# kasvii/PMCE

Measured on AMD Instinct MI355X. Metric: 16-frame clips/s, higher is better.
Workload: dtype f32; 1 GPU; full two-stream PMCE forward (temporal pose encoder + CoEvoDecoder + 6890-vertex upsample + J_regressor), batch=256/GPU, T=16, J=17, C=512, random-init weights; global_batch=256, seq_len=16, joints=17, embed_dim=512, parallelism=clip-sharded dp1, weights replicated, gemm_mode=split_f16, streams=4, batches_enqueued_ahead=2, lanes=staggered

## Files before the change

### pmce_amd/csrc/coevo.hip

```cpp
#include "common.hpp"

#define NV 431
#define ND 64
#define NTILE 14
#define LDW64 68
#define LDW256 260

__global__ __launch_bounds__(256) void vertex_init_gather_kernel(const float* __restrict__ joints,
                                                                 const int* __restrict__ vj, float* __restrict__ vt, int B,
                                                                 int J) {
  const int idx = blockIdx.x * blockDim.x + threadIdx.x;
  if (idx >= B * NV * 3) return;
  const int l = idx % 3, v = (idx / 3) % NV, b = idx / (3 * NV);
  vt[idx] = joints[((long long)b * J + vj[v]) * 3 + l];
}

#define JLD 65

#define JWL 68
#define JS_THREADS 512
struct JTile {
  f32x4 r[2];
};
__device__ __forceinline__ void jtile_fetch(JTile& t, const float* __restrict__ W, int ld, int n0, int k0, int tid) {
#pragma unroll
  for (int q = 0; q < 2; ++q) {
    const int row = (tid >> 4) + 32 * q, c4 = tid & 15;
    t.r[q] = *reinterpret_cast<const f32x4*>(W + (long long)(n0 + row) * ld + k0 + 4 * c4);
  }
}
__device__ __forceinline__ void jtile_store(float* s_w, const JTile& t, int tid) {
#pragma unroll
  for (int q = 0; q < 2; ++q) {
    const int row = (tid >> 4) + 32 * q, c4 = tid & 15;
    *reinterpret_cast<f32x4*>(s_w + row * JWL + 4 * c4) = t.r[q];
  }
}
template <int KIN, int NOUT>
__device__ __forceinline__ void lin_tiled(const float* in, int ild, const float* __restrict__ W, const float* __restrict__ b, float* out,
                                          int old, int J, int tid, bool gelu, float* s_w, JTile& pre, const float* __restrict__ Wnext,
                                          int ldnext) {
  constexpr int NT = NOUT / 64, KT = KIN / 64;
  const int lane = tid & 63, tg = tid >> 6;
#pragma unroll 1
  for (int nt = 0; nt < NT; ++nt) {
    float acc[4] = {0.f, 0.f, 0.f, 0.f};
    const int n = nt * 64 + lane;
    const float bn = b[n];
#pragma unroll 1
    for (int kt = 0; kt < KT; ++kt) {
      __syncthreads();
      jtile_store(s_w, pre, tid);
      __syncthreads();
      if (kt + 1 < KT) jtile_fetch(pre, W, KIN, nt * 64, (kt + 1) * 64, tid);
      else if (nt + 1 < NT) jtile_fetch(pre, W, KIN, (nt + 1) * 64, 0, tid);
      else if (Wnext) jtile_fetch(pre, Wnext, ldnext, 0, 0, tid);
      const float* wrow = s_w + lane * JWL;
#pragma unroll 4
      for (int k4 = 0; k4 < 16; ++k4) {
        const f32x4 wv = *reinterpret_cast<const f32x4*>(wrow + 4 * k4);
#pragma unroll
        for (int t = 0; t < 4; ++t) {
          const int i = tg + 8 * t;
          if (i < J) {
            const float* x = in + i * ild + kt * 64 + 4 * k4;
            acc[t] = fmaf(wv.x, x[0], acc[t]);
            acc[t] = fmaf(wv.y, x[1], acc[t]);
            acc[t] = fmaf(wv.z, x[2], acc[t]);
            acc[t] = fmaf(wv.w, x[3], acc[t]);
          }
        }
      }
    }
#pragma unroll
    for (int t = 0; t < 4; ++t) {
      const int i = tg + 8 * t;
      if (i < J) {
        const float v = acc[t] + bn;
        out[i * old + n] = gelu ? gelu_erf(v) : v;
      }
    }
  }
}
__device__ __forceinline__ void adaln_small8(const float* in, float* out, const float* __restrict__ gb, int J, int tid) {
  const int lane = tid & 63, wave = tid >> 6;
  const float gam = gb[lane], bet = gb[64 + lane];
  for (int i = wave; i < J; i += 8) {
    const float x = in[i * JLD + lane];
    const float mean = wave_sum(x) * (1.0f / 64.0f);
    const float d = x - mean;
    const float var = wave_sum(d * d) * (1.0f / 63.0f);
    float sd = sqrtf(var);
    if (var == INFINITY) {
      int e = 0;
      frexpf(wave_max(fabsf(d)), &e);
      const float ds = ldexpf(d, -e);
      sd = ldexpf(sqrtf(wave_sum(ds * ds) * (1.0f / 63.0f)), e);
    }
    out[i * JLD + lane] = gam * d / (sd + 1e-6f) + bet;
  }
}

#define CAM_VLD 52
#define CA_IMG_HDR 68
#define CA_IMG_FLOATS(J) (CA_IMG_HDR + 2 * (J) * LDW64 + 64 * CAM_VLD)
#define CA_IMG_STRIDE 6528
struct CaFoldArgs {
  const float *xk, *xv;
  const float *jt, *Wj, *bj, *jpos, *Wj2v, *bj2v, *j2vK;
  float* jf_out;
  const float* GB;
  int gb_stride, iq, ik, iv;
  const float *Wq, *bq, *Wk, *bk, *Wv, *bv, *Wp;
  float *Kf, *s0, *Vf;
  float* img;
  int J;
};
__global__ __launch_bounds__(JS_THREADS) void ca_fold_kernel(CaFoldArgs a) {
  __shared__ float s_a[32 * JLD];
  __shared__ float s_b[32 * JLD];
  __shared__ float s_k[32 * JLD];
  __shared__ float s_v[32 * JLD];
  __shared__ __attribute__((aligned(16))) float s_w[64 * JWL];
  __shared__ __attribute__((aligned(16))) float s_wp[64 * JWL];
  __shared__ __attribute__((aligned(16))) float s_img[CA_IMG_STRIDE];
  __shared__ float s_red[16];
  const int b = blockIdx.x, tid = threadIdx.x, lane = tid & 63, wave = tid >> 6;
  const int J = a.J;
  const float* gb = a.GB + (long long)b * a.gb_stride;
  JTile pre, prep;
  jtile_fetch(pre, a.xk ? a.Wk : a.Wj2v, 64, 0, 0, tid);
  jtile_fetch(prep, a.Wp, 64, 0, 0, tid);
  const float gq = gb[a.iq * 128 + lane], bqv = gb[a.iq * 128 + 64 + lane];
  if (a.img)
    for (int i = tid; i < CA_IMG_STRIDE; i += JS_THREADS) s_img[i] = 0.f;
  if (a.xk) {
    for (int idx = tid; idx < J * 64; idx += JS_THREADS) {
      const int i = idx >> 6, c = idx & 63;
      s_a[i * JLD + c] = a.xk[((long long)b * J + i) * 64 + c];
      s_b[i * JLD + c] = a.xv[((long long)b * J + i) * 64 + c];
    }
    jtile_store(s_wp, prep, tid);
    __syncthreads();
  } else {
    const int c = tid & 63, i0 = tid >> 6;
    const float w0 = a.Wj[c * 3], w1 = a.Wj[c * 3 + 1], w2 = a.Wj[c * 3 + 2], bjc = a.bj[c];
    float px[4], py[4], pz[4], pe[4], ke[4];
#pragma unroll
    for (int u = 0; u < 4; ++u) {
      const int i = i0 + 8 * u;
      if (i < J) {
        const float* p = a.jt + ((long long)b * J + i) * 3;
        px[u] = p[0]; py[u] = p[1]; pz[u] = p[2];
        pe[u] = a.jpos[i * 64 + c];
        ke[u] = a.j2vK[i * 64 + c];
      }
    }
#pragma unroll
    for (int u = 0; u < 4; ++u) {
      const int i = i0 + 8 * u;
      if (i < J) {
        const float v = ((w0 * px[u] + w1 * py[u] + w2 * pz[u]) + bjc) + pe[u];
        s_b[i * JLD + c] = v;
        if (a.jf_out) a.jf_out[((long long)b * J + i) * 64 + c] = v;
      }
    }
    jtile_store(s_wp, prep, tid);
    lin_tiled<64, 64>(s_b, JLD, a.Wj2v, a.bj2v, s_k, JLD, J, tid, false, s_w, pre, a.Wk, 64);
    __syncthreads();
#pragma unroll
    for (int u = 0; u < 4; ++u) {
      const int i = i0 + 8 * u;
      if (i < J) s_a[i * JLD + c] = s_k[i * JLD + c] + ke[u];
    }
    __syncthreads();
  }
  adaln_small8(s_a, s_k, gb + a.ik * 128, J, tid);
  adaln_small8(s_b, s_v, gb + a.iv * 128, J, tid);
  lin_tiled<64, 64>(s_k, JLD, a.Wk, a.bk, s_a, JLD, J, tid, false, s_w, pre, a.Wv, 64);
  lin_tiled<64, 64>(s_v, JLD, a.Wv, a.bv, s_b, JLD, J, tid, false, s_w, pre, a.Wq, 64);
  __syncthreads();
  jtile_store(s_w, pre, tid);
  __syncthreads();
  const float scale = 0.17677669529663688110f * 1.44269504088896340736f;
  float* Kfb = a.Kf ? a.Kf + (long long)b * 64 * 64 : nullptr;
  float* Vfb = a.Vf ? a.Vf + (long long)b * 64 * 64 : nullptr;
  float* s0b = a.s0 ? a.s0 + (long long)b * 64 : nullptr;
  float kfr[8], vfr[8];
  float mk = 0.f, mv = 0.f;
#pragma unroll
  for (int q8 = 0; q8 < 8; ++q8) {
    const int row = wave + 8 * q8;
    const int h = row >> 5, i = row & 31;
    float kf = 0.f, vf = 0.f, sc = 0.f;
    if (i < J) {
      float M = 0.f;
#pragma unroll
      for (int q = 0; q < 8; ++q) {
        const f32x4 wp4 = *reinterpret_cast<const f32x4*>(s_wp + lane * JWL + 32 * h + 4 * q);
        const float* kd = s_a + i * JLD + 32 * h + 4 * q;
        const float* vd = s_b + i * JLD + 32 * h + 4 * q;
        const float* wq = s_w + (32 * h + 4 * q) * JWL + lane;
        M += wq[0] * kd[0];
        vf += vd[0] * wp4.x;
        M += wq[JWL] * kd[1];
        vf += vd[1] * wp4.y;
        M += wq[2 * JWL] * kd[2];
        vf += vd[2] * wp4.z;
        M += wq[3 * JWL] * kd[3];
        vf += vd[3] * wp4.w;
      }
      kf = scale * gq * M;
      float t = bqv * M;
      if (lane < 32) t += a.bq[32 * h + lane] * s_a[i * JLD + 32 * h + lane];
      sc = scale * wave_sum(t);
    }
    if (Kfb) Kfb[row * 64 + lane] = kf;
    if (Vfb) Vfb[lane * 64 + row] = vf;
    if (s0b && lane == 0) s0b[row] = sc;
    if (a.img && lane == 0) s_img[row] = sc;
    kfr[q8] = kf;
    vfr[q8] = vf;
    mk = fmaxf(mk, fabsf(kf));
    mv = fmaxf(mv, fabsf(vf));
  }
  if (!a.img) return;
  mk = wave_max(mk);
  mv = wave_max(mv);
  if (lane == 0) {
    s_red[wave] = mk;
    s_red[8 + wave] = mv;
  }
  __syncthreads();
  float MK = 0.f, MV = 0.f;
#pragma unroll
  for (int w = 0; w < 8; ++w) {
    MK = fmaxf(MK, s_red[w]);
    MV = fmaxf(MV, s_red[8 + w]);
  }
  int ek = 0, ev = 0;
  const bool sk = MK > 0.f && MK < INFINITY, sv = MV > 0.f && MV < INFINITY;
  if (sk) frexpf(MK, &ek);
  if (sv) frexpf(MV, &ev);
  const float upK = sk ? ldexpf(1.f, 15 - ek) : 1.f, upV = sv ? ldexpf(1.f, 15 - ev) : 1.f;
  if (tid == 0) {
    s_img[64] = (sk ? ldexpf(1.f, ek - 15) : 1.f) * 0.0009765625f;
    s_img[65] = (sv ? ldexpf(1.f, ev - 15) : 1.f) * 0.0009765625f;
  }
  _Float16* im = reinterpret_cast<_Float16*>(s_img);
#pragma unroll
  for (int q8 = 0; q8 < 8; ++q8) {
    const int row = wave + 8 * q8;
    const int h = row >> 5, i = row & 31;
    if (i < J) {
      const float v = pinned(kfr[q8] * upK);
      const _Float16 hi = (_Float16)v, lo = (_Float16)(v - (float)hi);
      const int c = lane, ks = c >> 4, hbb = (c >> 2) & 1, e = (c & 3) + 4 * ((c >> 3) & 1);
      const int idx = (CA_IMG_HDR + (h * J + i) * LDW64) * 2 + ((ks * 2 + hbb) * 2) * 8 + e;
      im[idx] = hi;
      im[idx + 8] = lo;
    }
    if (i < 24) {
      const float v = pinned(vfr[q8] * upV);
      const _Float16 hi = (_Float16)v, lo = (_Float16)(v - (float)hi);
      const int base = (CA_IMG_HDR + 2 * J * LDW64 + lane * CAM_VLD) * 2 + h * 48;
      if (i < 16) {
        const int idx = base + ((i >> 2) & 1) * 16 + (i & 3) + 4 * (i >> 3);
        im[idx] = hi;
        im[idx + 8] = lo;
      } else {
        const int jj = i - 16;
        const int idx = base + 32 + (jj >> 2) * 8 + (jj & 3);
        im[idx] = hi;
        im[idx + 4] = lo;
      }
    }
  }
  __syncthreads();
  float* dst = a.img + (long long)b * CA_IMG_STRIDE;
  for (int i4 = tid; i4 < CA_IMG_FLOATS(J) / 4; i4 += JS_THREADS) reinterpret_cast<f32x4*>(dst)[i4] = reinterpret_cast<const f32x4*>(s_img)[i4];
}

__global__ __launch_bounds__(448, 4) void vertex_ca_kernel(const float* __restrict__ xq, const float* __restrict__ vt,
                                                        const float* __restrict__ Wv3, const float* __restrict__ Eq,
                                                        const float* __restrict__ Kf, const float* __restrict__ s0,
                                                        const float* __restrict__ Vf, const float* __restrict__ bp,
                                                        float* __restrict__ out, int J) {
  __shared__ __attribute__((aligned(16))) float sK[64 * LDW64];
  __shared__ __attribute__((aligned(16))) float sV[64 * LDW64];
  __shared__ float sS0[64];
  const int b = blockIdx.y, tid = threadIdx.x;
  const int lane = tid & 63, wave = tid >> 6;
  const int n0 = lane & 31, hb = lane >> 5;
  const int tile = blockIdx.x * 7 + wave;
// ... 1191 lines not shown
        }
#pragma unroll
        for (int r = 0; r < 16; ++r) y[16 * nt + r] = fmaf(fmaf(c[r], 0.00048828125f, m[r]), down, add[16 * nt + r]);
      }
    } else {
      f32x16 t[2];
#pragma unroll
      for (int nt = 0; nt < 2; ++nt)
#pragma unroll
        for (int r = 0; r < 16; ++r) t[nt][r] = add[16 * nt + r];
      tl_gemm<8, 2, LDW64>(sw, x, t, n0, hb);
#pragma unroll
      for (int nt = 0; nt < 2; ++nt)
#pragma unroll
        for (int r = 0; r < 16; ++r) y[16 * nt + r] = t[nt][r];
    }
  };
  for (int wt = blockIdx.x * 4 + wave; wt < ntiles; wt += gridDim.x * 4) {
    const int b = wt / NTILE, tile = wt % NTILE;
    const int v = tile * 32 + n0;
    const bool valid = v < NV;
    const int vc = valid ? v : NV - 1;
    const long long tok = (long long)b * NV + vc;
    float xk[32], xv[32];
    if (xk_in) {
      load_slots(xk_in + tok * 64, xk, hb);
      load_slots(xv_in + tok * 64, xv, hb);
    } else {
      const float* p = vt + tok * 3;
      const float p0 = p[0], p1 = p[1], p2 = p[2];
      load_slots(Ev + (long long)vc * 64, xv, hb);
#pragma unroll
      for (int s = 0; s < 32; ++s) {
        const int c = slot_channel(s, hb);
        xv[s] = (Wv3[c * 3] * p0 + Wv3[c * 3 + 1] * p1 + Wv3[c * 3 + 2] * p2) + xv[s];
      }
      float e[32];
      load_slots(Ek + (long long)vc * 64, e, hb);
      linear64(sW2, 0, xv, e, xk);
    }
    const float* gb = GB + (long long)b * gb_stride;
    float a[32], bias[32], y[32];
    adaln_slots(xk, a, gb + ik * 128, hb);
#pragma unroll
    for (int s = 0; s < 32; ++s) bias[s] = bk[slot_channel(s, hb)];
    linear64(sWk, 1, a, bias, y);
    if (valid) store_slots(kv + tok * 128, y, hb);
    adaln_slots(xv, a, gb + iv * 128, hb);
#pragma unroll
    for (int s = 0; s < 32; ++s) bias[s] = bv[slot_channel(s, hb)];
    linear64(sWv, 2, a, bias, y);
    if (valid) store_slots(kv + tok * 128 + 64, y, hb);
  }
}
__global__ __launch_bounds__(256) void tkv_pack_kernel(const float* __restrict__ W2, const float* __restrict__ Wk, const float* __restrict__ Wv,
                                                       float* __restrict__ img) {
  __shared__ float red[16];
  const float* W[3] = {W2, Wk, Wv};
  for (int i = 0; i < 3; ++i) {
    float up, down;
    weight_scale(W[i], 64 * 64, red, threadIdx.x, 256, up, down);
    stage_weight_split<64>(img + i * 64 * LDW64, W[i], 64, up, threadIdx.x, 256);
    if (threadIdx.x == 0) {
      img[3 * 64 * LDW64 + 2 * i] = up;
      img[3 * 64 * LDW64 + 2 * i + 1] = down;
    }
  }
}

struct JointStreamW {
  const float *wq, *bq, *proj_w, *proj_b;
  const float *fc1_w, *fc1_b, *fc2_w, *fc2_b;
  const float *qkv_w, *qkv_b, *sproj_w, *sproj_b;
  const float *sfc1_w, *sfc1_b, *sfc2_w, *sfc2_b;
  const float *coor_w, *coor_b;
  int i_normq, i_norm2, i_snorm1, i_snorm2;
};

__global__ __launch_bounds__(JS_THREADS) void joint_stream_kernel(const float* __restrict__ xq_in, const float* __restrict__ jQ,
                                                                  const float* __restrict__ kv, const float* __restrict__ GB,
                                                                  int gb_stride, JointStreamW w, const float* __restrict__ jt,
                                                                  float* __restrict__ y_out, float* __restrict__ pose_out, int J,
                                                                  int stage) {
  __shared__ float s_y[32 * JLD];
  __shared__ float s_a[32 * JLD];
  __shared__ float s_q[32 * JLD];
  __shared__ __attribute__((aligned(16))) float s_h[32 * 257];
  __shared__ __attribute__((aligned(16))) float s_kv[64 * 128];
  __shared__ __attribute__((aligned(16))) float s_w[64 * JWL];
  __shared__ float s_gb[4 * 128];
  __shared__ float s_cw[3 * 64 + 3];
  const int b = blockIdx.x, tid = threadIdx.x;
  {
    const float* gbg = GB + (long long)b * gb_stride;
    const int inst = tid >> 7, c = tid & 127;
    const int ii = inst == 0 ? w.i_normq : inst == 1 ? w.i_norm2 : inst == 2 ? w.i_snorm1 : w.i_snorm2;
    s_gb[inst * 128 + c] = gbg[ii * 128 + c];
    if (tid < 192) s_cw[tid] = w.coor_w[tid];
    if (tid < 3) s_cw[192 + tid] = w.coor_b[tid];
  }
  JTile pre;
  if (stage != 4) jtile_fetch(pre, w.wq, 64, 0, 0, tid);
  else jtile_fetch(pre, w.qkv_w, 64, 0, 0, tid);
  for (int idx = tid; idx < J * 64; idx += JS_THREADS) {
    const int i = idx >> 6, c = idx & 63;
    float v = xq_in[((long long)b * J + i) * 64 + c];
    if (jQ) v += jQ[i * 64 + c];
    s_y[i * JLD + c] = v;
  }
  __syncthreads();
  if (stage != 4) {
    adaln_small8(s_y, s_a, s_gb + 0 * 128, J, tid);
    lin_tiled<64, 64>(s_a, JLD, w.wq, w.bq, s_q, JLD, J, tid, false, s_w, pre, w.proj_w, 64);
    __syncthreads();
    {
      const int P = J * 8, NSL = JS_THREADS / P;
      const int pr = tid % P, sl = tid / P;
      const int i = pr >> 3, h = pr & 7;
      const bool act = sl < NSL;
      float qv[8], o[8];
      const float scale = 0.35355339059327376220f * 1.44269504088896340736f;
#pragma unroll
      for (int d = 0; d < 8; ++d) {
        qv[d] = act ? s_q[i * JLD + 8 * h + d] * scale : 0.f;
        o[d] = 0.f;
      }
      float m = -INFINITY, l = 0.f;
      const float* kvb = kv + (long long)b * NV * 128;
      f32x4 kvr[4];
      auto kv_fetch = [&](int j0) {
        const int nj = min(64, NV - j0);
#pragma unroll
        for (int q = 0; q < 4; ++q) {
          const int idx = tid + q * JS_THREADS, r = idx >> 5, c4 = idx & 31;
          if (r < nj) kvr[q] = *reinterpret_cast<const f32x4*>(kvb + (long long)(j0 + r) * 128 + 4 * c4);
        }
      };
      kv_fetch(0);
      for (int j0 = 0; j0 < NV; j0 += 64) {
        const int nj = min(64, NV - j0);
        __syncthreads();
#pragma unroll
        for (int q = 0; q < 4; ++q) {
          const int idx = tid + q * JS_THREADS, r = idx >> 5, c4 = idx & 31;
          if (r < nj) *reinterpret_cast<f32x4*>(&s_kv[r * 128 + 4 * c4]) = kvr[q];
        }
        __syncthreads();
        if (j0 + 64 < NV) kv_fetch(j0 + 64);
        if (act) {
          for (int r0 = sl; r0 < nj; r0 += 4 * NSL) {
            float sc[4];
#pragma unroll
            for (int u = 0; u < 4; ++u) {
              const int r = r0 + u * NSL;
              if (r < nj) {
                const f32x4 k0 = *reinterpret_cast<const f32x4*>(&s_kv[r * 128 + 8 * h]);
                const f32x4 k1 = *reinterpret_cast<const f32x4*>(&s_kv[r * 128 + 8 * h + 4]);
                sc[u] = qv[0] * k0.x + qv[1] * k0.y + qv[2] * k0.z + qv[3] * k0.w + qv[4] * k1.x + qv[5] * k1.y + qv[6] * k1.z +
                        qv[7] * k1.w;
              } else {
                sc[u] = -INFINITY;
              }
            }
            const float mn = fmaxf(fmaxf(m, fmaxf(sc[0], sc[1])), fmaxf(sc[2], sc[3]));
            const float corr = __builtin_amdgcn_exp2f(m - mn);
            l *= corr;
#pragma unroll
            for (int d = 0; d < 8; ++d) o[d] *= corr;
#pragma unroll
            for (int u = 0; u < 4; ++u) {
              const int r = r0 + u * NSL;
              if (r < nj) {
                const float pj = __builtin_amdgcn_exp2f(sc[u] - mn);
                l += pj;
                const f32x4 v0 = *reinterpret_cast<const f32x4*>(&s_kv[r * 128 + 64 + 8 * h]);
                const f32x4 v1 = *reinterpret_cast<const f32x4*>(&s_kv[r * 128 + 64 + 8 * h + 4]);
                o[0] += pj * v0.x;
                o[1] += pj * v0.y;
                o[2] += pj * v0.z;
                o[3] += pj * v0.w;
                o[4] += pj * v1.x;
                o[5] += pj * v1.y;
                o[6] += pj * v1.z;
                o[7] += pj * v1.w;
              }
            }
            m = mn;
          }
        }
      }
      if (act) {
        float* st = s_h + (sl * P + pr) * 10;
        st[0] = m;
        st[1] = l;
#pragma unroll
        for (int d = 0; d < 8; ++d) st[2 + d] = o[d];
      }
      __syncthreads();
      if (act && sl == 0) {
        float M = m;
        for (int s2 = 1; s2 < NSL; ++s2) M = fmaxf(M, s_h[(s2 * P + pr) * 10]);
        float L = 0.f, O[8] = {0.f, 0.f, 0.f, 0.f, 0.f, 0.f, 0.f, 0.f};
        for (int s2 = 0; s2 < NSL; ++s2) {
          const float* st = s_h + (s2 * P + pr) * 10;
          const float c = __builtin_amdgcn_exp2f(st[0] - M);
          L += st[1] * c;
#pragma unroll
          for (int d = 0; d < 8; ++d) O[d] += st[2 + d] * c;
        }
        const float inv = 1.0f / L;
#pragma unroll
        for (int d = 0; d < 8; ++d) s_a[i * JLD + 8 * h + d] = O[d] * inv;
      }
    }
    lin_tiled<64, 64>(s_a, JLD, w.proj_w, w.proj_b, s_q, JLD, J, tid, false, s_w, pre, stage == 1 ? nullptr : w.fc1_w, 64);
    __syncthreads();
    for (int idx = tid; idx < J * 64; idx += JS_THREADS) {
      const int i = idx >> 6, c = idx & 63;
      s_y[i * JLD + c] += s_q[i * JLD + c];
    }
    __syncthreads();
    if (stage == 1) {
      for (int idx = tid; idx < J * 64; idx += JS_THREADS) y_out[(long long)b * J * 64 + idx] = s_y[(idx >> 6) * JLD + (idx & 63)];
      return;
    }
    adaln_small8(s_y, s_a, s_gb + 1 * 128, J, tid);
    lin_tiled<64, 256>(s_a, JLD, w.fc1_w, w.fc1_b, s_h, 257, J, tid, true, s_w, pre, w.fc2_w, 256);
    lin_tiled<256, 64>(s_h, 257, w.fc2_w, w.fc2_b, s_q, JLD, J, tid, false, s_w, pre, stage == 2 ? nullptr : w.qkv_w, 64);
    __syncthreads();
    for (int idx = tid; idx < J * 64; idx += JS_THREADS) {
      const int i = idx >> 6, c = idx & 63;
      s_y[i * JLD + c] += s_q[i * JLD + c];
    }
    __syncthreads();
    if (stage == 2) {
      for (int idx = tid; idx < J * 64; idx += JS_THREADS) y_out[(long long)b * J * 64 + idx] = s_y[(idx >> 6) * JLD + (idx & 63)];
      return;
    }
  }
  adaln_small8(s_y, s_a, s_gb + 2 * 128, J, tid);
  lin_tiled<64, 192>(s_a, JLD, w.qkv_w, w.qkv_b, s_h, 193, J, tid, false, s_w, pre, w.sproj_w, 64);
  __syncthreads();
  {
    const int i = tid >> 3, h = tid & 7;
    if (i < J) {
      const float scale = 0.35355339059327376220f * 1.44269504088896340736f;
      float qv[8], o[8];
#pragma unroll
      for (int d = 0; d < 8; ++d) {
        qv[d] = s_h[i * 193 + 8 * h + d] * scale;
        o[d] = 0.f;
      }
      float m = -INFINITY, l = 0.f;
      for (int j = 0; j < J; ++j) {
        float sc = 0.f;
#pragma unroll
        for (int d = 0; d < 8; ++d) sc += qv[d] * s_h[j * 193 + 64 + 8 * h + d];
        const float mn = fmaxf(m, sc);
        const float corr = __builtin_amdgcn_exp2f(m - mn), pj = __builtin_amdgcn_exp2f(sc - mn);
        l = l * corr + pj;
#pragma unroll
        for (int d = 0; d < 8; ++d) o[d] = o[d] * corr + pj * s_h[j * 193 + 128 + 8 * h + d];
        m = mn;
      }
      const float inv = 1.0f / l;
#pragma unroll
      for (int d = 0; d < 8; ++d) s_a[i * JLD + 8 * h + d] = o[d] * inv;
    }
  }
  lin_tiled<64, 64>(s_a, JLD, w.sproj_w, w.sproj_b, s_q, JLD, J, tid, false, s_w, pre, w.sfc1_w, 64);
  __syncthreads();
  for (int idx = tid; idx < J * 64; idx += JS_THREADS) {
    const int i = idx >> 6, c = idx & 63;
    s_y[i * JLD + c] += s_q[i * JLD + c];
  }
  __syncthreads();
  adaln_small8(s_y, s_a, s_gb + 3 * 128, J, tid);
  lin_tiled<64, 256>(s_a, JLD, w.sfc1_w, w.sfc1_b, s_h, 257, J, tid, true, s_w, pre, w.sfc2_w, 256);
  lin_tiled<256, 64>(s_h, 257, w.sfc2_w, w.sfc2_b, s_q, JLD, J, tid, false, s_w, pre, nullptr, 0);
  __syncthreads();
  for (int idx = tid; idx < J * 64; idx += JS_THREADS) {
    const int i = idx >> 6, c = idx & 63;
    s_y[i * JLD + c] += s_q[i * JLD + c];
  }
  __syncthreads();
  if (y_out)
    for (int idx = tid; idx < J * 64; idx += JS_THREADS) y_out[(long long)b * J * 64 + idx] = s_y[(idx >> 6) * JLD + (idx & 63)];
  if (pose_out) {
    for (int idx = tid; idx < J * 3; idx += JS_THREADS) {
      const int i = idx / 3, k = idx % 3;
      float s = 0.f;
      for (int c = 0; c < 64; ++c) s += s_cw[k * 64 + c] * s_y[i * JLD + c];
      pose_out[((long long)b * J + i) * 3 + k] = (s + s_cw[192 + k]) + jt[((long long)b * J + i) * 3 + k];
    }
  }
}

template <bool PACKED>
__global__ __launch_bounds__(256) void build_final_operand_kernel(const float* __restrict__ g, const float* __restrict__ vt,
                                                                  float* __restrict__ A, int B, int KP) {
  const long long idx = (long long)blockIdx.x * blockDim.x + threadIdx.x;
  if (idx >= (long long)B * KP) return;
  const int b = (int)(idx / KP), k = (int)(idx % KP);
  float v = 0.f;
  if (k < 2048)
    v = fmaxf(g[(long long)b * 2048 + k], 0.f);
  else if (k < 2048 + NV * 3)
    v = vt[(long long)b * NV * 3 + (k - 2048)];
  if constexpr (PACKED) {
    _Float16* row = reinterpret_cast<_Float16*>(A + (long long)b * KP);
    const _Float16 h = (_Float16)v;
    row[(k >> 4) * 32 + (k & 15)] = h;
    row[(k >> 4) * 32 + 16 + (k & 15)] = lo_plane_plain(v, h);
  } else {
    A[idx] = v;
  }
}

__global__ __launch_bounds__(256) void j_regress_kernel(const float* __restrict__ mesh, const int* __restrict__ indptr,
                                                        const int* __restrict__ indices, const float* __restrict__ data,
                                                        float* __restrict__ out, int B, int R, int NVF, float scale) {
  const int idx = blockIdx.x * blockDim.x + threadIdx.x;
  if (idx >= B * R * 3) return;
  const int l = idx % 3, j = (idx / 3) % R, b = idx / (3 * R);
  const float* m = mesh + (long long)b * NVF * 3;
  float s = 0.f;
  for (int e = indptr[j]; e < indptr[j + 1]; ++e) s += data[e] * (m[(long long)indices[e] * 3 + l] * scale);
  out[idx] = s;
}

#define MLP_WAVES 8
#define CAM_WAVES 7
static int mlp_grid(int B) {
  const int tiles = B * NTILE;
  int g = (tiles + MLP_WAVES - 1) / MLP_WAVES;
  return g < 256 ? g : 256;
}
static int tl_grid(int B, int per_cu) {
  const int tiles = B * NTILE;
  int g = (tiles + 3) / 4;
  const int cap = 256 * per_cu;
  return g < cap ? g : cap;
}

extern "C" int pmce_vertex_init_gather_f32(const float* joints, const int* vj, float* vt, int B, int J, hipStream_t stream) {
  PMCE_REQUIRE(joints && vj && vt && B > 0 && J > 0, "vertex_init_gather: bad args");
  const int n = B * NV * 3;
  hipLaunchKernelGGL(vertex_init_gather_kernel, dim3((n + 255) / 256), dim3(256), 0, stream, joints, vj, vt, B, J);
  return pmce_check_launch("vertex_init_gather");
}

static int launch_ca_fold(const CaFoldArgs& a, int B, hipStream_t stream, const char* what) {
  PMCE_REQUIRE(a.J >= 1 && a.J <= 32 && B > 0, "%s: J must be in 1..32", what);
  PMCE_REQUIRE(!a.img || (a.J <= 23 && (reinterpret_cast<uintptr_t>(a.img) & 15) == 0), "%s: the f16 image needs J <= 23 and a 16-byte aligned buffer", what);
  hipLaunchKernelGGL(ca_fold_kernel, dim3(B), dim3(JS_THREADS), 0, stream, a);
  return pmce_check_launch(what);
}
extern "C" int pmce_ca_image_floats(void) { return CA_IMG_STRIDE; }
extern "C" int pmce_ca_image_floats_written(int J) { return CA_IMG_FLOATS(J); }
extern "C" int pmce_ca_fold_f32(const float* xk, const float* xv, const float* GB, int gb_stride, int iq, int ik, int iv,
                                const float* Wq, const float* bq, const float* Wk, const float* bk, const float* Wv,
                                const float* bv, const float* Wp, float* Kf, float* s0, float* Vf, float* img, int B, int J,
                                hipStream_t stream) {
  PMCE_REQUIRE(xk && xv && GB && Wq && bq && Wk && bk && Wv && bv && Wp, "ca_fold: null pointer");
  CaFoldArgs a{};
  a.xk = xk; a.xv = xv; a.GB = GB; a.gb_stride = gb_stride; a.iq = iq; a.ik = ik; a.iv = iv;
  a.Wq = Wq; a.bq = bq; a.Wk = Wk; a.bk = bk; a.Wv = Wv; a.bv = bv; a.Wp = Wp;
// ... 186 lines not shown
```

Before: 30570 clips/s.

## Move joint-stream linears to FP32 MFMA with async LDS weight DMA

Swaps the scalar-FMA tiled linear layers in the cross-attention fold and joint-stream kernels for 32x32x2 FP32 MFMA tiles. Full weight matrices are prefetched into LDS through buffer-load-to-LDS DMA ahead of use, replacing the register-staged tile double buffering. The FFN keeps its hidden activations in registers and feeds them straight into the second GEMM. K-split partial sums are reduced in shared memory with the bias and residual fused in. The LDS is reorganised into one aliased arena and token rows are padded to 32 with zeros, which raises LDS footprint and could lower occupancy.

After: 30740 clips/s (median of 6 runs). No clear change (+0.6%).

```diff
diff --git a/pmce_amd/csrc/coevo.hip b/pmce_amd/csrc/coevo.hip
--- a/pmce_amd/csrc/coevo.hip
+++ b/pmce_amd/csrc/coevo.hip
@@ -15,70 +15,88 @@
   vt[idx] = joints[((long long)b * J + vj[v]) * 3 + l];
 }
 
-#define JLD 65
+#define JLD 68
 
 #define JWL 68
+#define JWL4 260
 #define JS_THREADS 512
-struct JTile {
-  f32x4 r[2];
-};
-__device__ __forceinline__ void jtile_fetch(JTile& t, const float* __restrict__ W, int ld, int n0, int k0, int tid) {
-#pragma unroll
-  for (int q = 0; q < 2; ++q) {
-    const int row = (tid >> 4) + 32 * q, c4 = tid & 15;
-    t.r[q] = *reinterpret_cast<const f32x4*>(W + (long long)(n0 + row) * ld + k0 + 4 * c4);
-  }
-}
-__device__ __forceinline__ void jtile_store(float* s_w, const JTile& t, int tid) {
-#pragma unroll
-  for (int q = 0; q < 2; ++q) {
-    const int row = (tid >> 4) + 32 * q, c4 = tid & 15;
-    *reinterpret_cast<f32x4*>(s_w + row * JWL + 4 * c4) = t.r[q];
-  }
-}
-template <int KIN, int NOUT>
-__device__ __forceinline__ void lin_tiled(const float* in, int ild, const float* __restrict__ W, const float* __restrict__ b, float* out,
-                                          int old, int J, int tid, bool gelu, float* s_w, JTile& pre, const float* __restrict__ Wnext,
-                                          int ldnext) {
-  constexpr int NT = NOUT / 64, KT = KIN / 64;
-  const int lane = tid & 63, tg = tid >> 6;
-#pragma unroll 1
-  for (int nt = 0; nt < NT; ++nt) {
-    float acc[4] = {0.f, 0.f, 0.f, 0.f};
-    const int n = nt * 64 + lane;
+#define JW_SLOT (64 * JWL)
+template <int KIN>
+__device__ __forceinline__ void jl_dma_rows(float* lds_dst, const float* __restrict__ W, int rows, int tid) {
+  constexpr int CPR = KIN / 4 + 1;
+  const __amdgpu_buffer_rsrc_t rsrc = __builtin_amdgcn_make_buffer_rsrc(const_cast<float*>(W), 0, 0xffffffff, 0x00020000);
+  const unsigned base = __builtin_amdgcn_readfirstlane((unsigned)(uintptr_t)(const __attribute__((address_space(3))) float*)lds_dst);
+  const int w0 = __builtin_amdgcn_readfirstlane(tid >> 6), lane = tid & 63;
+  const int pieces = rows * CPR / 64;
+  for (int c = w0; c < pieces; c += JS_THREADS / 64) {
+    const int g = c * 64 + lane, row = g / CPR, col = min(g % CPR, CPR - 2);
+    lds_dma16(rsrc, (unsigned)((row * KIN + 4 * col) * 4), 0, base + (unsigned)c * 1024u);
+  }
+}
+template <int NQ>
+__device__ __forceinline__ void jl_mma(f32x16& acc, const float* Wrow, const float* xrow) {
+#pragma unroll
+  for (int q = 0; q < NQ; ++q) {
+    const f32x4 wv = *reinterpret_cast<const f32x4*>(Wrow + 8 * q);
+    const f32x4 xv = *reinterpret_cast<const f32x4*>(xrow + 8 * q);
+    acc = __builtin_amdgcn_mfma_f32_32x32x2f32(wv.x, xv.x, acc, 0, 0, 0);
+    acc = __builtin_amdgcn_mfma_f32_32x32x2f32(wv.y, xv.y, acc, 0, 0, 0);
+    acc = __builtin_amdgcn_mfma_f32_32x32x2f32(wv.z, xv.z, acc, 0, 0, 0);
+    acc = __builtin_amdgcn_mfma_f32_32x32x2f32(wv.w, xv.w, acc, 0, 0, 0);
+  }
+}
+__device__ __forceinline__ f32x16 jl_zero() {
+  f32x16 z;
+#pragma unroll
+  for (int r = 0; r < 16; ++r) z[r] = 0.f;
+  return z;
+}
+__device__ __forceinline__ void jl_store_part(float* part, int nb, const f32x16& acc, int lane) {
+  const int tok = lane & 31, hb = lane >> 5;
+#pragma unroll
+  for (int r = 0; r < 16; ++r) part[(32 * nb + (r & 3) + 8 * (r >> 2) + 4 * hb) * 32 + tok] = acc[r];
+}
+__device__ __forceinline__ void jl_lin64_parts(const float* in, const float* Wl, float* parts, int tid) {
+  const int lane = tid & 63, wave = tid >> 6, n = lane & 31, hb = lane >> 5;
+  const int nb = wave & 1, kq = wave >> 1;
+  f32x16 acc = jl_zero();
+  jl_mma<2>(acc, Wl + (32 * nb + n) * JWL + 16 * kq + 4 * hb, in + n * JLD + 16 * kq + 4 * hb);
+  jl_store_part(parts + kq * 2048, nb, acc, lane);
+}
+template <int NP>
+__device__ __forceinline__ void jl_meet(const float* parts, const float* __restrict__ b, float* out, bool residual, int J, int tid) {
+#pragma unroll
+  for (int u = 0; u < 4; ++u) {
+    const int o = tid + JS_THREADS * u, n = o >> 5, tok = o & 31;
     const float bn = b[n];
-#pragma unroll 1
-    for (int kt = 0; kt < KT; ++kt) {
-      __syncthreads();
-      jtile_store(s_w, pre, tid);
-      __syncthreads();
-      if (kt + 1 < KT) jtile_fetch(pre, W, KIN, nt * 64, (kt + 1) * 64, tid);
-      else if (nt + 1 < NT) jtile_fetch(pre, W, KIN, (nt + 1) * 64, 0, tid);
-      else if (Wnext) jtile_fetch(pre, Wnext, ldnext, 0, 0, tid);
-      const float* wrow = s_w + lane * JWL;
-#pragma unroll 4
-      for (int k4 = 0; k4 < 16; ++k4) {
-        const f32x4 wv = *reinterpret_cast<const f32x4*>(wrow + 4 * k4);
-#pragma unroll
-        for (int t = 0; t < 4; ++t) {
-          const int i = tg + 8 * t;
-          if (i < J) {
-            const float* x = in + i * ild + kt * 64 + 4 * k4;
-            acc[t] = fmaf(wv.x, x[0], acc[t]);
-            acc[t] = fmaf(wv.y, x[1], acc[t]);
-            acc[t] = fmaf(wv.z, x[2], acc[t]);
-            acc[t] = fmaf(wv.w, x[3], acc[t]);
-          }
-        }
-      }
-    }
-#pragma unroll
-    for (int t = 0; t < 4; ++t) {
-      const int i = tg + 8 * t;
-      if (i < J) {
-        const float v = acc[t] + bn;
-        out[i * old + n] = gelu ? gelu_erf(v) : v;
-      }
+    float s = parts[o];
+#pragma unroll
+    for (int p = 1; p < NP; ++p) s += parts[p * 2048 + o];
+    const float v = s + bn;
+    if (tok < J) out[tok * JLD + n] = residual ? out[tok * JLD + n] + v : v;
+  }
+}
+__device__ __forceinline__ void jl_ffn_parts(const float* in, const float* W1l, const float* W2l, const float* __restrict__ b1, f32x16* acc2,
+                                             int tid) {
+  const int lane = tid & 63, wave = tid >> 6, n = lane & 31, hb = lane >> 5;
+  float bv[16];
+#pragma unroll
+  for (int r = 0; r < 16; ++r) bv[r] = b1[32 * wave + (r & 3) + 8 * (r >> 2) + 4 * hb];
+  f32x16 h = jl_zero();
+  jl_mma<8>(h, W1l + (32 * wave + n) * JWL + 4 * hb, in + n * JLD + 4 * hb);
+#pragma unroll
+  for (int r = 0; r < 16; ++r) h[r] = gelu_erf(h[r] + bv[r]);
+#pragma unroll
+  for (int nb = 0; nb < 2; ++nb) {
+    acc2[nb] = jl_zero();
+    const float* Wrow = W2l + (32 * nb + n) * JWL4 + 32 * wave + 4 * hb;
+#pragma unroll
+    for (int q = 0; q < 4; ++q) {
+      const f32x4 wv = *reinterpret_cast<const f32x4*>(Wrow + 8 * q);
+      acc2[nb] = __builtin_amdgcn_mfma_f32_32x32x2f32(wv.x, h[4 * q + 0], acc2[nb], 0, 0, 0);
+      acc2[nb] = __builtin_amdgcn_mfma_f32_32x32x2f32(wv.y, h[4 * q + 1], acc2[nb], 0, 0, 0);
+      acc2[nb] = __builtin_amdgcn_mfma_f32_32x32x2f32(wv.z, h[4 * q + 2], acc2[nb], 0, 0, 0);
+      acc2[nb] = __builtin_amdgcn_mfma_f32_32x32x2f32(wv.w, h[4 * q + 3], acc2[nb], 0, 0, 0);
     }
   }
 }
@@ -117,30 +135,36 @@
   int J;
 };
 __global__ __launch_bounds__(JS_THREADS) void ca_fold_kernel(CaFoldArgs a) {
-  __shared__ float s_a[32 * JLD];
-  __shared__ float s_b[32 * JLD];
-  __shared__ float s_k[32 * JLD];
-  __shared__ float s_v[32 * JLD];
-  __shared__ __attribute__((aligned(16))) float s_w[64 * JWL];
-  __shared__ __attribute__((aligned(16))) float s_wp[64 * JWL];
-  __shared__ __attribute__((aligned(16))) float s_img[CA_IMG_STRIDE];
-  __shared__ float s_red[16];
+  __shared__ __attribute__((aligned(16))) float smem[4 * 32 * JLD + 5 * JW_SLOT + 2 * JW_SLOT + 16];
+  float* s_a = smem;
+  float* s_b = s_a + 32 * JLD;
+  float* s_k = s_b + 32 * JLD;
+  float* s_v = s_k + 32 * JLD;
+  float* s_wt = s_v + 32 * JLD;
+  float* s_wq = s_wt + 3 * JW_SLOT;
+  float* s_wp = s_wt + 4 * JW_SLOT;
+  float* s_parts = s_wt + 5 * JW_SLOT;
+  float* s_M = s_parts;
+  float* s_VF = s_parts + JW_SLOT;
+  float* s_red = s_parts + 2 * JW_SLOT;
+  float* s_img = s_wt;
   const int b = blockIdx.x, tid = threadIdx.x, lane = tid & 63, wave = tid >> 6;
   const int J = a.J;
   const float* gb = a.GB + (long long)b * a.gb_stride;
-  JTile pre, prep;
-  jtile_fetch(pre, a.xk ? a.Wk : a.Wj2v, 64, 0, 0, tid);
-  jtile_fetch(prep, a.Wp, 64, 0, 0, tid);
+  if (!a.xk) jl_dma_rows<64>(s_wt, a.Wj2v, 64, tid);
+  jl_dma_rows<64>(s_wt + JW_SLOT, a.Wk, 64, tid);
+  jl_dma_rows<64>(s_wt + 2 * JW_SLOT, a.Wv, 64, tid);
+  jl_dma_rows<64>(s_wq, a.Wq, 64, tid);
+  jl_dma_rows<64>(s_wp, a.Wp, 64, tid);
   const float gq = gb[a.iq * 128 + lane], bqv = gb[a.iq * 128 + 64 + lane];
-  if (a.img)
-    for (int i = tid; i < CA_IMG_STRIDE; i += JS_THREADS) s_img[i] = 0.f;
   if (a.xk) {
-    for (int idx = tid; idx < J * 64; idx += JS_THREADS) {
+    for (int idx = tid; idx < 32 * 64; idx += JS_THREADS) {
       const int i = idx >> 6, c = idx & 63;
-      s_a[i * JLD + c] = a.xk[((long long)b * J + i) * 64 + c];
-      s_b[i * JLD + c] = a.xv[((long long)b * J + i) * 64 + c];
-    }
-    jtile_store(s_wp, prep, tid);
+      s_a[i * JLD + c] = i < J ? a.xk[((long long)b * J + i) * 64 + c] : 0.f;
+      s_b[i * JLD + c] = i < J ? a.xv[((long long)b * J + i) * 64 + c] : 0.f;
+      s_k[i * JLD + c] = 0.f;
+      s_v[i * JLD + c] = 0.f;
+    }
     __syncthreads();
   } else {
     const int c = tid & 63, i0 = tid >> 6;
@@ -159,14 +183,21 @@
 #pragma unroll
     for (int u = 0; u < 4; ++u) {
       const int i = i0 + 8 * u;
+      float v = 0.f;
       if (i < J) {
-        const float v = ((w0 * px[u] + w1 * py[u] + w2 * pz[u]) + bjc) + pe[u];
-        s_b[i * JLD + c] = v;
+        v = ((w0 * px[u] + w1 * py[u] + w2 * pz[u]) + bjc) + pe[u];
         if (a.jf_out) a.jf_out[((long long)b * J + i) * 64 + c] = v;
       }
-    }
-    jtile_store(s_wp, prep, tid);
-    lin_tiled<64, 64>(s_b, JLD, a.Wj2v, a.bj2v, s_k, JLD, J, tid, false, s_w, pre, a.Wk, 64);
+      s_b[i * JLD + c] = v;
+      s_a[i * JLD + c] = 0.f;
+      s_k[i * JLD + c] = 0.f;
+      s_v[i * JLD + c] = 0.f;
+    }
+    lds_dma_wait();
+    __syncthreads();
+    jl_lin64_parts(s_b, s_wt, s_parts, tid);
+    __syncthreads();
+    jl_meet<4>(s_parts, a.bj2v, s_k, false, J, tid);
     __syncthreads();
 #pragma unroll
     for (int u = 0; u < 4; ++u) {
@@ -177,10 +208,38 @@
   }
   adaln_small8(s_a, s_k, gb + a.ik * 128, J, tid);
   adaln_small8(s_b, s_v, gb + a.iv * 128, J, tid);
-  lin_tiled<64, 64>(s_k, JLD, a.Wk, a.bk, s_a, JLD, J, tid, false, s_w, pre, a.Wv, 64);
-  lin_tiled<64, 64>(s_v, JLD, a.Wv, a.bv, s_b, JLD, J, tid, false, s_w, pre, a.Wq, 64);
-  __syncthreads();
-  jtile_store(s_w, pre, tid);
+  lds_dma_wait();
+  __syncthreads();
+  jl_lin64_parts(s_k, s_wt + JW_SLOT, s_parts, tid);
+  __syncthreads();
+  jl_meet<4>(s_parts, a.bk, s_a, false, J, tid);
+  __syncthreads();
+  jl_lin64_parts(s_v, s_wt + 2 * JW_SLOT, s_parts, tid);
+  __syncthreads();
+  jl_meet<4>(s_parts, a.bv, s_b, false, J, tid);
+  __syncthreads();
+  if (a.img)
+    for (int i = tid; i < CA_IMG_STRIDE; i += JS_THREADS) s_img[i] = 0.f;
+  {
+    const int n = lane & 31, hb = lane >> 5, kind = wave >> 2, h = (wave >> 1) & 1, cb = wave & 1, c = 32 * cb + n;
+    f32x16 acc = jl_zero();
+    if (kind == 0) {
+#pragma unroll
+      for (int q = 0; q < 4; ++q) {
+        const f32x4 xv = *reinterpret_cast<const f32x4*>(s_a + n * JLD + 32 * h + 8 * q + 4 * hb);
+        const float* wq = s_wq + (32 * h + 8 * q + 4 * hb) * JWL + c;
+        acc = __builtin_amdgcn_mfma_f32_32x32x2f32(wq[0], xv.x, acc, 0, 0, 0);
+        acc = __builtin_amdgcn_mfma_f32_32x32x2f32(wq[JWL], xv.y, acc, 0, 0, 0);
+        acc = __builtin_amdgcn_mfma_f32_32x32x2f32(wq[2 * JWL], xv.z, acc, 0, 0, 0);
+        acc = __builtin_amdgcn_mfma_f32_32x32x2f32(wq[3 * JWL], xv.w, acc, 0, 0, 0);
+      }
+    } else {
+      jl_mma<4>(acc, s_wp + c * JWL + 32 * h + 4 * hb, s_b + n * JLD + 32 * h + 4 * hb);
+    }
+    float* dst = (kind == 0 ? s_M : s_VF) + (32 * h + n) * JWL + 32 * cb + 4 * hb;
+#pragma unroll
+    for (int g = 0; g < 4; ++g) *reinterpret_cast<f32x4*>(dst + 8 * g) = f32x4{acc[4 * g], acc[4 * g + 1], acc[4 * g + 2], acc[4 * g + 3]};
+  }
   __syncthreads();
   const float scale = 0.17677669529663688110f * 1.44269504088896340736f;
   float* Kfb = a.Kf ? a.Kf + (long long)b * 64 * 64 : nullptr;
@@ -194,22 +253,8 @@
     const int h = row >> 5, i = row & 31;
     float kf = 0.f, vf = 0.f, sc = 0.f;
     if (i < J) {
-      float M = 0.f;
-#pragma unroll
-      for (int q = 0; q < 8; ++q) {
-        const f32x4 wp4 = *reinterpret_cast<const f32x4*>(s_wp + lane * JWL + 32 * h + 4 * q);
-        const float* kd = s_a + i * JLD + 32 * h + 4 * q;
-        const float* vd = s_b + i * JLD + 32 * h + 4 * q;
-        const float* wq = s_w + (32 * h + 4 * q) * JWL + lane;
-        M += wq[0] * kd[0];
-        vf += vd[0] * wp4.x;
-        M += wq[JWL] * kd[1];
-        vf += vd[1] * wp4.y;
-        M += wq[2 * JWL] * kd[2];
-        vf += vd[2] * wp4.z;
-        M += wq[3 * JWL] * kd[3];
-        vf += vd[3] * wp4.w;
-      }
+      const float M = s_M[row * JWL + lane];
+      vf = s_VF[row * JWL + lane];
       kf = scale * gq * M;
       float t = bqv * M;
       if (lane < 32) t += a.bq[32 * h + lane] * s_a[i * JLD + 32 * h + lane];
@@ -1567,15 +1612,25 @@
                                                                   int gb_stride, JointStreamW w, const float* __restrict__ jt,
                                                                   float* __restrict__ y_out, float* __restrict__ pose_out, int J,
                                                                   int stage) {
-  __shared__ float s_y[32 * JLD];
-  __shared__ float s_a[32 * JLD];
-  __shared__ float s_q[32 * JLD];
-  __shared__ __attribute__((aligned(16))) float s_h[32 * 257];
-  __shared__ __attribute__((aligned(16))) float s_kv[64 * 128];
-  __shared__ __attribute__((aligned(16))) float s_w[64 * JWL];
-  __shared__ float s_gb[4 * 128];
-  __shared__ float s_cw[3 * 64 + 3];
+  __shared__ __attribute__((aligned(16))) float smem[2 * 32 * JLD + 8 * JW_SLOT + 4 * 128 + 3 * 64 + 3];
+  float* s_y = smem;
+  float* s_a = s_y + 32 * JLD;
+  float* R1 = s_a + 32 * JLD;
+  float* R2 = R1 + 4 * JW_SLOT;
+  float* s_gb = R2 + 4 * JW_SLOT;
+  float* s_cw = s_gb + 4 * 128;
+  float* s_kv = R1;
+  float* s_q = R1 + 2 * JW_SLOT;
+  float* s_st = s_q + 32 * JLD;
+  float* s_qkv = R1;
   const int b = blockIdx.x, tid = threadIdx.x;
+  if (stage != 4) {
+    jl_dma_rows<64>(R2, w.wq, 64, tid);
+    jl_dma_rows<64>(R2 + JW_SLOT, w.proj_w, 64, tid);
+  } else {
+    jl_dma_rows<64>(R2, w.qkv_w, 192, tid);
+    jl_dma_rows<64>(R2 + 3 * JW_SLOT, w.sproj_w, 64, tid);
+  }
   {
     const float* gbg = GB + (long long)b * gb_stride;
     const int inst = tid >> 7, c = tid & 127;
@@ -1584,19 +1639,24 @@
     if (tid < 192) s_cw[tid] = w.coor_w[tid];
     if (tid < 3) s_cw[192 + tid] = w.coor_b[tid];
   }
-  JTile pre;
-  if (stage != 4) jtile_fetch(pre, w.wq, 64, 0, 0, tid);
-  else jtile_fetch(pre, w.qkv_w, 64, 0, 0, tid);
-  for (int idx = tid; idx < J * 64; idx += JS_THREADS) {
+  for (int idx = tid; idx < 32 * 64; idx += JS_THREADS) {
     const int i = idx >> 6, c = idx & 63;
-    float v = xq_in[((long long)b * J + i) * 64 + c];
-    if (jQ) v += jQ[i * 64 + c];
+    float v = 0.f;
+    if (i < J) {
+      v = xq_in[((long long)b * J + i) * 64 + c];
+      if (jQ) v += jQ[i * 64 + c];
+    }
     s_y[i * JLD + c] = v;
+    s_a[i * JLD + c] = 0.f;
   }
   __syncthreads();
   if (stage != 4) {
     adaln_small8(s_y, s_a, s_gb + 0 * 128, J, tid);
-    lin_tiled<64, 64>(s_a, JLD, w.wq, w.bq, s_q, JLD, J, tid, false, s_w, pre, w.proj_w, 64);
+    lds_dma_wait();
+    __syncthreads();
+    jl_lin64_parts(s_a, R2, R2 + 2 * JW_SLOT, tid);
+    __syncthreads();
+    jl_meet<4>(R2 + 2 * JW_SLOT, w.bq, s_q, false, J, tid);
     __syncthreads();
     {
       const int P = J * 8, NSL = JS_THREADS / P;
@@ -1675,7 +1735,7 @@
         }
       }
       if (act) {
-        float* st = s_h + (sl * P + pr) * 10;
+        float* st = s_st + (sl * P + pr) * 10;
         st[0] = m;
         st[1] = l;
 #pragma unroll
@@ -1684,10 +1744,10 @@
       __syncthreads();
       if (act && sl == 0) {
         float M = m;
-        for (int s2 = 1; s2 < NSL; ++s2) M = fmaxf(M, s_h[(s2 * P + pr) * 10]);
+        for (int s2 = 1; s2 < NSL; ++s2) M = fmaxf(M, s_st[(s2 * P + pr) * 10]);
         float L = 0.f, O[8] = {0.f, 0.f, 0.f, 0.f, 0.f, 0.f, 0.f, 0.f};
         for (int s2 = 0; s2 < NSL; ++s2) {
-          const float* st = s_h + (s2 * P + pr) * 10;
+          const float* st = s_st + (s2 * P + pr) * 10;
           const float c = __builtin_amdgcn_exp2f(st[0] - M);
           L += st[1] * c;
 #pragma unroll
@@ -1698,25 +1758,31 @@
         for (int d = 0; d < 8; ++d) s_a[i * JLD + 8 * h + d] = O[d] * inv;
       }
     }
-    lin_tiled<64, 64>(s_a, JLD, w.proj_w, w.proj_b, s_q, JLD, J, tid, false, s_w, pre, stage == 1 ? nullptr : w.fc1_w, 64);
     __syncthreads();
-    for (int idx = tid; idx < J * 64; idx += JS_THREADS) {
-      const int i = idx >> 6, c = idx & 63;
-      s_y[i * JLD + c] += s_q[i * JLD + c];
-    }
+    if (stage != 1) jl_dma_rows<64>(R1, w.fc1_w, 256, tid);
+    jl_lin64_parts(s_a, R2 + JW_SLOT, R2 + 2 * JW_SLOT, tid);
+    __syncthreads();
+    jl_meet<4>(R2 + 2 * JW_SLOT, w.proj_b, s_y, true, J, tid);
     __syncthreads();
     if (stage == 1) {
       for (int idx = tid; idx < J * 64; idx += JS_THREADS) y_out[(long long)b * J * 64 + idx] = s_y[(idx >> 6) * JLD + (idx & 63)];
       return;
     }
+    jl_dma_rows<256>(R2, w.fc2_w, 64, tid);
     adaln_small8(s_y, s_a, s_gb + 1 * 128, J, tid);
-    lin_tiled<64, 256>(s_a, JLD, w.fc1_w, w.fc1_b, s_h, 257, J, tid, true, s_w, pre, w.fc2_w, 256);
-    lin_tiled<256, 64>(s_h, 257, w.fc2_w, w.fc2_b, s_q, JLD, J, tid, false, s_w, pre, stage == 2 ? nullptr : w.qkv_w, 64);
+    lds_dma_wait();
     __syncthreads();
-    for (int idx = tid; idx < J * 64; idx += JS_THREADS) {
-      const int i = idx >> 6, c = idx & 63;
-      s_y[i * JLD + c] += s_q[i * JLD + c];
-    }
+    f32x16 acc2[2];
+    jl_ffn_parts(s_a, R1, R2, w.fc1_b, acc2, tid);
+    __syncthreads();
+    if (stage != 2) {
+      jl_dma_rows<64>(R2, w.qkv_w, 192, tid);
+      jl_dma_rows<64>(R2 + 3 * JW_SLOT, w.sproj_w, 64, tid);
+    }
+    jl_store_part(R1 + (tid >> 6) * 2048, 0, acc2[0], tid & 63);
+    jl_store_part(R1 + (tid >> 6) * 2048, 1, acc2[1], tid & 63);
+    __syncthreads();
+    jl_meet<8>(R1, w.fc2_b, s_y, true, J, tid);
     __syncthreads();
     if (stage == 2) {
       for (int idx = tid; idx < J * 64; idx += JS_THREADS) y_out[(long long)b * J * 64 + idx] = s_y[(idx >> 6) * JLD + (idx & 63)];
@@ -1724,7 +1790,22 @@
     }
   }
   adaln_small8(s_y, s_a, s_gb + 2 * 128, J, tid);
-  lin_tiled<64, 192>(s_a, JLD, w.qkv_w, w.qkv_b, s_h, 193, J, tid, false, s_w, pre, w.sproj_w, 64);
+  lds_dma_wait();
+  __syncthreads();
+  if (tid < 6 * 64) {
+    const int lane = tid & 63, wave = tid >> 6, n = lane & 31, hb = lane >> 5;
+    float bv[16];
+#pragma unroll
+    for (int r = 0; r < 16; ++r) bv[r] = w.qkv_b[32 * wave + (r & 3) + 8 * (r >> 2) + 4 * hb];
+    f32x16 acc = jl_zero();
+    jl_mma<8>(acc, R2 + (32 * wave + n) * JWL + 4 * hb, s_a + n * JLD + 4 * hb);
+    if (n < J) {
+#pragma unroll
+      for (int g = 0; g < 4; ++g)
+        *reinterpret_cast<f32x4*>(s_qkv + n * 196 + 32 * wave + 8 * g + 4 * hb) =
+            f32x4{acc[4 * g] + bv[4 * g], acc[4 * g + 1] + bv[4 * g + 1], acc[4 * g + 2] + bv[4 * g + 2], acc[4 * g + 3] + bv[4 * g + 3]};
+    }
+  }
   __syncthreads();
   {
     const int i = tid >> 3, h = tid & 7;
@@ -1733,19 +1814,19 @@
       float qv[8], o[8];
 #pragma unroll
       for (int d = 0; d < 8; ++d) {
-        qv[d] = s_h[i * 193 + 8 * h + d] * scale;
+        qv[d] = s_qkv[i * 196 + 8 * h + d] * scale;
         o[d] = 0.f;
       }
       float m = -INFINITY, l = 0.f;
       for (int j = 0; j < J; ++j) {
         float sc = 0.f;
 #pragma unroll
-        for (int d = 0; d < 8; ++d) sc += qv[d] * s_h[j * 193 + 64 + 8 * h + d];
+        for (int d = 0; d < 8; ++d) sc += qv[d] * s_qkv[j * 196 + 64 + 8 * h + d];
         const float mn = fmaxf(m, sc);
         const float corr = __builtin_amdgcn_exp2f(m - mn), pj = __builtin_amdgcn_exp2f(sc - mn);
         l = l * corr + pj;
 #pragma unroll
-        for (int d = 0; d < 8; ++d) o[d] = o[d] * corr + pj * s_h[j * 193 + 128 + 8 * h + d];
+        for (int d = 0; d < 8; ++d) o[d] = o[d] * corr + pj * s_qkv[j * 196 + 128 + 8 * h + d];
         m = mn;
       }
       const float inv = 1.0f / l;
@@ -1753,21 +1834,25 @@
       for (int d = 0; d < 8; ++d) s_a[i * JLD + 8 * h + d] = o[d] * inv;
     }
   }
-  lin_tiled<64, 64>(s_a, JLD, w.sproj_w, w.sproj_b, s_q, JLD, J, tid, false, s_w, pre, w.sfc1_w, 64);
-  __syncthreads();
-  for (int idx = tid; idx < J * 64; idx += JS_THREADS) {
-    const int i = idx >> 6, c = idx & 63;
-    s_y[i * JLD + c] += s_q[i * JLD + c];
-  }
-  __syncthreads();
+  __syncthreads();
+  jl_dma_rows<64>(R1, w.sfc1_w, 256, tid);
+  jl_lin64_parts(s_a, R2 + 3 * JW_SLOT, R2, tid);
+  __syncthreads();
+  jl_meet<4>(R2, w.sproj_b, s_y, true, J, tid);
+  __syncthreads();
+  jl_dma_rows<256>(R2, w.sfc2_w, 64, tid);
   adaln_small8(s_y, s_a, s_gb + 3 * 128, J, tid);
-  lin_tiled<64, 256>(s_a, JLD, w.sfc1_w, w.sfc1_b, s_h, 257, J, tid, true, s_w, pre, w.sfc2_w, 256);
-  lin_tiled<256, 64>(s_h, 257, w.sfc2_w, w.sfc2_b, s_q, JLD, J, tid, false, s_w, pre, nullptr, 0);
-  __syncthreads();
-  for (int idx = tid; idx < J * 64; idx += JS_THREADS) {
-    const int i = idx >> 6, c = idx & 63;
-    s_y[i * JLD + c] += s_q[i * JLD + c];
-  }
+  lds_dma_wait();
+  __syncthreads();
+  {
+    f32x16 acc2[2];
+    jl_ffn_parts(s_a, R1, R2, w.sfc1_b, acc2, tid);
+    __syncthreads();
+    jl_store_part(R1 + (tid >> 6) * 2048, 0, acc2[0], tid & 63);
+    jl_store_part(R1 + (tid >> 6) * 2048, 1, acc2[1], tid & 63);
+  }
+  __syncthreads();
+  jl_meet<8>(R1, w.sfc2_b, s_y, true, J, tid);
   __syncthreads();
   if (y_out)
     for (int idx = tid; idx < J * 64; idx += JS_THREADS) y_out[(long long)b * J * 64 + idx] = s_y[(idx >> 6) * JLD + (idx & 63)];
```
